# MKimiSH/video-filler

Hardware: AMD Instinct MI355X
Metric: netG+netD fwd+bwd images/sec, 128x128 center-mask (higher is better)
Workload: dtype f32

## Files before the change

video-filler_amd/csrc/vf_conv.hip:

```cpp
#include <algorithm>
#include <vector>
#include <cstdlib>

#include "vf_device.h"

template <int LD>
__device__ __forceinline__ bf16x8 vf_tr_frag(const __bf16* tile, int col0, int k0, int lane) {
  const int grp = lane >> 4, i = lane & 15;
  const __bf16* a = tile + (k0 + 8 * (grp >> 1) + (i >> 2)) * LD + col0 + 16 * (grp & 1) + 4 * (i & 3);
  typedef __attribute__((address_space(3))) bf16x4 lds_bf16x4;
  const bf16x4 lo = __builtin_amdgcn_ds_read_tr16_b64_v4bf16((lds_bf16x4*)a);
  const bf16x4 hi = __builtin_amdgcn_ds_read_tr16_b64_v4bf16((lds_bf16x4*)(a + 4 * LD));
  return __builtin_shufflevector(lo, hi, 0, 1, 2, 3, 4, 5, 6, 7);
}

struct IGemm {
  const float* A;
  const float* Wt;
  const float* bias;
  float* Y;
  float* slab;
  int64_t out_elems;
  unsigned a_bytes, w_bytes;
  int M, lgMh, lgMw;
// ... 1302 lines not shown
  VF_REQUIRE((s.stride == 2 && s.pad == 1) || (s.stride == 1 && s.pad == 0), "unsupported stride/pad %d/%d", s.stride, s.pad);
  VF_REQUIRE(s.B > 0 && s.Cin > 0 && s.Cout > 0, "bad sizes B=%d Cin=%d Cout=%d", s.B, s.Cin, s.Cout);
  VF_REQUIRE(s.pow2_map(), "spatial sizes must be powers of two (got %dx%d)", s.H, s.W);
  if (s.stride == 1) VF_REQUIRE(s.H >= 4 && s.W >= 4, "4x4 stride-1 conv needs H,W >= 4");
  if (s.stride == 2) VF_REQUIRE(s.H >= 2 && s.W >= 2, "stride-2 conv needs H,W >= 2");
  VF_REQUIRE((int64_t)s.Cin * s.Cout * 16 < ((int64_t)1 << 31), "weight tensor too large for 32-bit element offsets");
  return 0;
}
static int check_full_conv_args(const VfConvShape& s) {
  VF_REQUIRE(s.main_net_taps(), "unsupported full-conv shape");
  VF_REQUIRE(s.pow2_map(), "spatial sizes must be powers of two");
  return 0;
}

static int conv_like_fwd(vf_ctx* ctx, const float* A, const float* w, const float* bias, float* Y, const VfConvShape& s, int act,
                         float slope, VfConvExtras* ex) {
  const int B = s.B, Hi = s.H, Wi = s.W, C = s.Cin, N = s.Cout, stride = s.stride, pad = s.pad, Ho = s.out_h(), Wo = s.out_w();
  VF_REQUIRE(vf_is_pow2(Ho) && vf_is_pow2(Wo), "output spatial sizes must be powers of two");
  if (N == 1 && stride == 1 && Hi == 4 && Wi == 4) {
    hipLaunchKernelGGL(k_dot_fwd, dim3(B), dim3(256), 0, ctx->stream, A, w, bias, Y, 16 * C, act, slope);
    VF_LAUNCH_CHECK();
    return 0;
  }
  IGemm g;
  memset(&g, 0, sizeof(g));
  g.A = A; g.Wt = w; g.bias = bias; g.Y = Y;
  g.lgMh = vf_ilog2(Ho); g.lgMw = vf_ilog2(Wo);
  g.M = B * Ho * Wo;
  g.Hi = Hi; g.Wi = Wi; g.C = C; g.N = N;
  g.TH = 4; g.TW = 4;
  g.sy = stride; g.ty = 1; g.oy0 = -pad; g.sx = stride; g.tx = 1; g.ox0 = -pad;
  g.kh0 = 0; g.khs = 1; g.kw0 = 0; g.kws = 1;
  g.wsN = 16 * C; g.wsC = 1; g.wsTap = C;
  g.outH = Ho; g.outW = Wo; g.osy = 1; g.osx = 1;
  g.out_elems = (int64_t)g.M * N;
  g.act = act; g.slope = slope;
  return launch_igemm(ctx, g, (C % 16 == 0) && vf_aligned16(A), (C % 16 == 0) && vf_aligned16(w), ex);
}

static int conv_like_bwd(vf_ctx* ctx, const float* A, const float* w, const float* bias, float* Y, const VfConvShape& s, int act,
                         float slope, VfConvExtras* ex, const float* dmask = nullptr, int dact = 0, float dslope = 0.f) {
  const int B = s.B, Hi = s.H, Wi = s.W, C = s.Cin, N = s.Cout, stride = s.stride, pad = s.pad;
  if (stride == 2 && pad == 1 && N <= 4 && !dmask && !ex->bn.st.mode) {
    const int rc = vf_internal_deconv_thin_out(ctx, A, w, bias, Y, s, act, slope);
    if (rc >= 0) return rc;
  }
  IGemm g;
  memset(&g, 0, sizeof(g));
  g.A = A; g.Wt = w; g.bias = bias; g.Y = Y;
  g.dmask = dmask; g.dact = dact; g.dslope = dslope;
  g.Hi = Hi; g.Wi = Wi; g.C = C; g.N = N;
  g.wsN = 1; g.wsC = 16 * N; g.wsTap = N;
  g.act = act; g.slope = slope;
  const bool vecA = (C % 16 == 0) && vf_aligned16(A);
  bool vecB = (N % 4 == 0) && vf_aligned16(w);
  if (stride == 2 && N < 32 && vecA && vf_aligned16(w) && ctx->ws_front == 0) {
    const int64_t Mi = (int64_t)B * Hi * Wi;
    const size_t col_bytes = (size_t)Mi * 16 * N * sizeof(float);
    if (col_bytes + ((size_t)32 << 20) <= ctx->ws_bytes) {
      float* cols = (float*)ctx->ws;
      ctx->ws_front = (col_bytes + 255) & ~(size_t)255;
      IGemm q;
      memset(&q, 0, sizeof(q));
      q.A = A; q.Wt = w; q.bias = nullptr; q.Y = cols;
      q.M = (int)Mi; q.lgMh = 0; q.lgMw = 0;
      q.Hi = 1; q.Wi = 1; q.C = C; q.N = 16 * N;
      q.TH = 1; q.TW = 1; q.sy = 1; q.ty = 1; q.sx = 1; q.tx = 1; q.khs = 1; q.kws = 1;
      q.wsN = 1; q.wsC = 16 * N; q.wsTap = 0;
      q.outH = 1; q.outW = 1; q.osy = 1; q.osx = 1;
      q.out_elems = Mi * 16 * N;
      q.act = VF_ACT_NONE;
      const int rc = launch_igemm(ctx, q, true, true, nullptr);
      ctx->ws_front = 0;
      if (rc) return rc;
      const int64_t total = Mi * 4 * N;
      VfProf prof(ctx, "col2im4x4", 0.0, 4.0 * ((double)Mi * 16 * N + (double)total));
      hipLaunchKernelGGL(k_col2im4x4, dim3((unsigned)vf_cdiv(total, 256)), dim3(256), 0, ctx->stream, (const float*)cols, bias, Y,
                         B, vf_ilog2(Hi), vf_ilog2(Wi), N, act, slope);
      VF_LAUNCH_CHECK();
      if (dmask) return vf_act_bwd(ctx, dmask, Y, Y, total, dact, dslope);
      return 0;
    }
  }
  if (stride == 2) {
    g.lgMh = vf_ilog2(Hi); g.lgMw = vf_ilog2(Wi);
    g.M = B * Hi * Wi;
    g.TH = 2; g.TW = 2;
    g.sy = 1; g.ty = -1; g.oy0 = 0; g.sx = 1; g.tx = -1; g.ox0 = 0;
    g.khs = 2; g.kws = 2;
    g.outH = 2 * Hi; g.outW = 2 * Wi; g.osy = 2; g.osx = 2;
    g.parity = 1;
    g.out_elems = (int64_t)B * g.outH * g.outW * N;
  } else {
    VF_REQUIRE(Hi == 1 && Wi == 1, "stride-1 transposed pass is built for the 1x1 bottleneck only (got %dx%d)", Hi, Wi);
    g.lgMh = 0; g.lgMw = 0;
    g.M = B;
    g.TH = 1; g.TW = 1;
    g.sy = 1; g.ty = 1; g.sx = 1; g.tx = 1;
    g.N = 16 * N;
    g.wsC = 16 * N; g.wsTap = 0;
    g.outH = 1; g.outW = 1; g.osy = 1; g.osx = 1;
    g.out_elems = (int64_t)B * 16 * N;
    vecB = ((16 * N) % 4 == 0) && vf_aligned16(w);
  }
  VF_REQUIRE(!(dmask && bias), "activation-backward epilogue is for data-gradient passes (no bias)");
  if (stride == 1 && bias) {
    g.bias = nullptr;
    g.act = VF_ACT_NONE;
  }
  if (int rc = launch_igemm(ctx, g, vecA, vecB, stride == 2 ? ex : nullptr)) return rc;
  if (stride == 1 && bias) {
    const int64_t total = (int64_t)B * 16 * N;
    const int nb = (int)std::min<int64_t>(vf_cdiv(total, 256), 4096);
    hipLaunchKernelGGL(k_slab_reduce, dim3(nb), dim3(256), 0, ctx->stream, (const float*)Y, Y, bias, total, N, 0, act, slope, 1.f);
    VF_LAUNCH_CHECK();
  }
  return 0;
}

struct WgRec {
  WGrad g;
  int bm, bf;
  VfPWGrad pw;
  bool plain_ok;
  int blocks;
  int64_t total;
  double flops;
};
struct WgRecorder {
  std::vector<WgRec> recs;
  size_t ws_used = 0;
};
void vf_internal_wg_free(vf_ctx* ctx) {
  delete (WgRecorder*)ctx->wg_rec;
  ctx->wg_rec = nullptr;
}
template <int BM, int BF>
static void launch_wg_group(vf_ctx* ctx, const WGradGroup& G, int blocks, const char* name, double flops) {
  VF_LAUNCH_TIMED(ctx, name, flops, 0.0, (k_wgrad_group<BM, true, true, BF>), dim3(blocks), dim3(256), G);
}
static int wg_flush(vf_ctx* ctx) {
  WgRecorder* R = (WgRecorder*)ctx->wg_rec;
  if (!R || R->recs.empty()) return 0;
  {
    bool any_planes = false;
    for (const WgRec& r : R->recs) any_planes |= (r.bf == 4);
    if (any_planes)
      for (WgRec& r : R->recs)
        if ((r.bf == 3 || r.bf == 1) && r.plain_ok) {
          r.bf = 4;
          r.blocks = r.pw.gx * r.pw.gy;
        }
    VfPWGradGroup G;
    int blocks = 0;
    double fl = 0;
    G.n = 0;
    auto fire = [&]() -> int {
      if (G.n == 0) return 0;
      G.blk_off[G.n] = blocks;
      const int rc = vf_internal_pwgrad_group(ctx, G, blocks, "pwgrad_group_128x128x32", fl);
      G.n = 0;
      blocks = 0;
      fl = 0;
      return rc;
    };
    for (const WgRec& r : R->recs) {
      if (r.bf != 4) continue;
      G.blk_off[G.n] = blocks;
      G.d[G.n] = r.pw;
      ++G.n;
      blocks += (r.blocks + 7) & ~7;
      fl += r.flops;
      if (G.n == VF_PWG_MAX)
        if (int rc = fire()) return rc;
    }
    if (int rc = fire()) return rc;
  }
  for (int bm : {128, 64})
    for (int bf : {3, 1, 0}) {
      WGradGroup G;
      int blocks = 0;
      double fl = 0;
      G.n = 0;
      auto fire = [&]() {
        if (G.n == 0) return;
        G.blk_off[G.n] = blocks;
        char name[64];
        snprintf(name, sizeof(name), "wgrad_group_%dx128%s", bm, bf == 3 ? "_bf16x3" : (bf ? "_bf16" : ""));
        if (bm == 128) {
          if (bf == 3) launch_wg_group<128, 3>(ctx, G, blocks, name, fl);
          else if (bf == 1) launch_wg_group<128, 1>(ctx, G, blocks, name, fl);
          else launch_wg_group<128, 0>(ctx, G, blocks, name, fl);
        } else {
          if (bf == 3) launch_wg_group<64, 3>(ctx, G, blocks, name, fl);
          else if (bf == 1) launch_wg_group<64, 1>(ctx, G, blocks, name, fl);
          else launch_wg_group<64, 0>(ctx, G, blocks, name, fl);
        }
        G.n = 0;
        blocks = 0;
        fl = 0;
      };
      for (const WgRec& r : R->recs) {
        if (r.bm != bm || r.bf != bf) continue;
        G.blk_off[G.n] = blocks;
        G.d[G.n] = r.g;
        ++G.n;
        blocks += (r.blocks + 7) & ~7;
        fl += r.flops;
        if (G.n == VF_WG_GROUP_MAX) fire();
      }
      fire();
    }
  VF_LAUNCH_CHECK();
  {
    SlabGroup S;
    int blocks = 0;
    double bytes = 0;
    S.n = 0;
    auto fire = [&]() {
      if (S.n == 0) return;
      S.blk_off[S.n] = blocks;
      VfProf prof(ctx, "slab_reduce_wgrad_group", 0.0, bytes);
      hipLaunchKernelGGL(k_slab_reduce4_group, dim3(blocks), dim3(256), 0, ctx->stream, S);
      S.n = 0;
      blocks = 0;
      bytes = 0;
    };
    for (const WgRec& r : R->recs) {
      if (r.g.ksplit <= 1) continue;
      S.blk_off[S.n] = blocks;
      S.d[S.n].slab = r.g.slab;
      S.d[S.n].dst = r.g.dW;
      S.d[S.n].total4 = r.total / 4;
      S.d[S.n].ksplit = r.g.ksplit;
      S.d[S.n].beta = r.g.beta;
      ++S.n;
      blocks += (int)vf_cdiv(r.total / 4, 64);
      bytes += 4.0 * (double)r.total * (r.g.ksplit + 1);
      if (S.n == VF_WG_GROUP_MAX) fire();
    }
    fire();
  }
  VF_LAUNCH_CHECK();
  R->recs.clear();
  R->ws_used = 0;
  return 0;
}
VF_API int vf_wgrad_group_begin(vf_ctx* ctx) {
  if (!ctx->wg_rec) ctx->wg_rec = new WgRecorder();
  if (ctx->wg_active) {
    ((WgRecorder*)ctx->wg_rec)->recs.clear();
    ((WgRecorder*)ctx->wg_rec)->ws_used = 0;
  }
  ctx->wg_active = 1;
  return 0;
}
VF_API int vf_wgrad_group_abort(vf_ctx* ctx) {
  if (ctx->wg_rec) {
    ((WgRecorder*)ctx->wg_rec)->recs.clear();
    ((WgRecorder*)ctx->wg_rec)->ws_used = 0;
  }
  ctx->wg_active = 0;
  return 0;
}
VF_API int vf_wgrad_group_end(vf_ctx* ctx) {
  VF_REQUIRE(ctx->wg_active, "vf_wgrad_group_end: no group is open");
  ctx->wg_active = 0;
  return wg_flush(ctx);
}

VF_API int vf_wgrad_group_count(vf_ctx* ctx, int* count) {
  VF_REQUIRE(count != nullptr, "vf_wgrad_group_count: NULL");
  *count = (ctx->wg_active && ctx->wg_rec) ? (int)((WgRecorder*)ctx->wg_rec)->recs.size() : 0;
  return 0;
}
VF_API int vf_wgrad_group_end_partial(vf_ctx* ctx, int count) {
  VF_REQUIRE(ctx->wg_active, "vf_wgrad_group_end_partial: no group is open");
  WgRecorder* R = (WgRecorder*)ctx->wg_rec;
  if (!R || R->recs.empty() || count <= 0) return 0;
  if (count >= (int)R->recs.size()) {
    const size_t used = R->ws_used;
    const int rc = wg_flush(ctx);
    R->ws_used = used;
    return rc;
  }
  std::vector<WgRec> rest(R->recs.begin() + count, R->recs.end());
  R->recs.resize((size_t)count);
  const size_t used = R->ws_used;
  const int rc = wg_flush(ctx);
  R->recs = rest;
  R->ws_used = used;
  return rc;
}

static int wgrad(vf_ctx* ctx, const float* U, const float* V, float* dW, const VfConvShape& s, bool full, float beta, const void* Up,
                 const void* Vp) {
  const int B = s.B, stride = s.stride, pad = s.pad, ntaps = 16;
  const int Hl = full ? s.H : s.out_h(), Wl = full ? s.W : s.out_w(), Nu = full ? s.Cin : s.Cout;
  const int Hv = full ? s.full_out_h() : s.H, Wv = full ? s.full_out_w() : s.W, Cv = full ? s.Cout : s.Cin;
  if (Hl == 1 && Wl == 1 && Hv == 4 && Wv == 4 && stride == 1 && pad == 0 && ntaps == 16) {
    const int rc = vf_internal_wgrad_smallk(ctx, U, V, dW, B, Nu, 16 * Cv, beta);
    if (rc >= 0) return rc;
  }
  WGrad g;
  memset(&g, 0, sizeof(g));
  g.U = U; g.V = V; g.dW = dW;
  g.P = B * Hl * Wl;
  g.lgMh = vf_ilog2(Hl); g.lgMw = vf_ilog2(Wl);
  g.Nu = Nu; g.Cv = Cv; g.Hv = Hv; g.Wv = Wv;
  g.stride = stride; g.pad = pad;
  g.ntaps = ntaps;
  g.nk = (int)vf_cdiv(g.P, ctx->mfma_bf16 ? 32 : 16);
  VF_REQUIRE((int64_t)g.P * Nu < ((int64_t)1 << 29) && (int64_t)B * Hv * Wv * Cv < ((int64_t)1 << 29),
             "operand exceeds the 2 GiB buffer-descriptor range");
  g.u_bytes = (unsigned)((int64_t)g.P * Nu * 4);
  g.v_bytes = (unsigned)((int64_t)B * Hv * Wv * Cv * 4);
  const bool vecU = (Nu % 4 == 0) && vf_aligned16(U);
  const bool vecV = (Cv % 4 == 0) && vf_aligned16(V);
  g.beta = beta;
  const int BM = Nu > 64 ? 128 : 64;
  const int gy = (int)vf_cdiv(Nu, BM), gx = (int)vf_cdiv(ntaps * (int64_t)Cv, 128);
  const int64_t blocks = (int64_t)gx * gy;
  const int64_t total = (int64_t)Nu * ntaps * Cv;
  int ksplit = 1;
  const bool use_pw = Up && Vp && (ctx->mfma_bf16 == 3 || ctx->mfma_bf16 == 1) && ntaps == 16 && stride == 2 && pad == 1 && Nu % 128 == 0 &&
                      Cv % 64 == 0 && g.P % 32 == 0 && (int64_t)g.P * Nu * 6 < ((int64_t)1 << 31) &&
                      (int64_t)B * Hv * Wv * Cv * 6 < ((int64_t)1 << 31) && total % 4 == 0;
  const int wg_blocks = use_pw ? 256 : 512;
  if (blocks < wg_blocks * 3 / 4 && g.nk >= 16) {
    ksplit = (int)std::min<int64_t>(g.nk / 8, vf_cdiv(wg_blocks, blocks));
    while (ksplit > 1 && (size_t)ksplit * total * sizeof(float) > vf_ws_avail(ctx)) --ksplit;
    if (ksplit < 1) ksplit = 1;
    const int steps = (int)vf_cdiv(g.nk, ksplit);
    ksplit = (int)vf_cdiv(g.nk, steps);
  }
  g.ksplit = ksplit;
  g.slab = ksplit > 1 ? (float*)vf_ws_ptr(ctx) : nullptr;
  g.gx = gx; g.gy = gy; g.gz = ksplit;
  dim3 grid((unsigned)gx * gy * ksplit), block(256);
  const bool own_group = use_pw && !ctx->wg_active;
  if (own_group) {
    if (!ctx->wg_rec) ctx->wg_rec = new WgRecorder();
    ctx->wg_active = 1;
  }
  if (ctx->wg_active && (use_pw || (vecU && vecV && (ksplit == 1 || total % 4 == 0)))) {
    WgRecorder* R = (WgRecorder*)ctx->wg_rec;
    const size_t need = ksplit > 1 ? (((size_t)ksplit * total * sizeof(float) + 255) & ~(size_t)255) : 0;
    if (R->ws_used + need > vf_ws_avail(ctx)) {
      if (int rc = wg_flush(ctx)) return rc;
      R->ws_used = 0;
    }
    VF_REQUIRE(need <= vf_ws_avail(ctx), "workspace too small for this layer's split-K slabs");
    if (ksplit > 1) g.slab = (float*)(vf_ws_ptr(ctx) + R->ws_used);
    R->ws_used += need;
    WgRec r;
    r.g = g;
    r.bm = BM;
    r.bf = ctx->mfma_bf16;
    r.blocks = gx * gy * ksplit;
    r.total = total;
    r.flops = 2.0 * (double)g.P * Nu * (double)ntaps * Cv;
    r.plain_ok = false;
    if (!use_pw && (ctx->mfma_bf16 == 3 || ctx->mfma_bf16 == 1) && BM == 128 && ksplit == 1 && Hl == 1 && Wl == 1 && Hv == 4 && Wv == 4 && stride == 1 &&
        pad == 0 && ntaps == 16 && Nu % 4 == 0 && (16 * Cv) % 128 == 0 && vecU && vecV) {
      r.plain_ok = true;
      VfPWGrad& w = r.pw;
      memset(&w, 0, sizeof(w));
      w.Uf = U; w.Vf = V;
      w.out = dW;
      w.P = g.P; w.Nu = Nu; w.Cv = Cv; w.Hv = Hv; w.Wv = Wv;
      w.gx = (16 * Cv) / 128; w.gy = (int)vf_cdiv(Nu, 128); w.gz = 1;
      w.ksplit = 1; w.nk = (int)vf_cdiv(g.P, 32);
      w.beta = beta;
    }
    if (use_pw) {
      r.bf = 4;
      VfPWGrad& w = r.pw;
      memset(&w, 0, sizeof(w));
      w.Up = Up; w.Vp = Vp;
      w.out = ksplit > 1 ? g.slab : dW;
      w.u_ps = (unsigned)((int64_t)g.P * Nu * 2);
      w.v_ps = (unsigned)((int64_t)B * Hv * Wv * Cv * 2);
      w.P = g.P; w.lgMh = g.lgMh; w.lgMw = g.lgMw;
      w.Nu = Nu; w.Cv = Cv; w.Hv = Hv; w.Wv = Wv;
      w.gx = gx; w.gy = gy; w.gz = ksplit;
      w.ksplit = ksplit; w.nk = g.nk;
      w.beta = beta;
    }
    R->recs.push_back(r);
    if (own_group) {
      ctx->wg_active = 0;
      return wg_flush(ctx);
    }
    return 0;
  }
  if (ctx->wg_active) {
    WgRecorder* R = (WgRecorder*)ctx->wg_rec;
    const size_t need = ksplit > 1 ? (((size_t)ksplit * total * sizeof(float) + 255) & ~(size_t)255) : 0;
    if (R && R->ws_used + need <= vf_ws_avail(ctx)) {
      if (ksplit > 1) g.slab = (float*)(vf_ws_ptr(ctx) + R->ws_used);
      R->ws_used += need;
    } else if (int rc = wg_flush(ctx)) {
      return rc;
    }
  }
  {
    const int bf = ctx->mfma_bf16;
    const char* wname = BM == 128 ? (bf == 3 ? "wgrad_128x128_bf16x3" : bf ? "wgrad_128x128_bf16" : "wgrad_128x128")
                                  : (bf == 3 ? "wgrad_64x128_bf16x3" : bf ? "wgrad_64x128_bf16" : "wgrad_64x128");
    const double wfl = 2.0 * (double)g.P * Nu * (double)ntaps * Cv;
#define VF_WG(BM_, BF_)                                                                              \
  do {                                                                                              \
    if (vecU && vecV)                                                                               \
      VF_LAUNCH_TIMED(ctx, wname, wfl, 0.0, (k_wgrad<BM_, true, true, BF_>), grid, block, g);       \
    else if (vecU)                                                                                  \
      VF_LAUNCH_TIMED(ctx, wname, wfl, 0.0, (k_wgrad<BM_, true, false, BF_>), grid, block, g);      \
    else if (vecV)                                                                                  \
      VF_LAUNCH_TIMED(ctx, wname, wfl, 0.0, (k_wgrad<BM_, false, true, BF_>), grid, block, g);      \
    else                                                                                            \
      VF_LAUNCH_TIMED(ctx, wname, wfl, 0.0, (k_wgrad<BM_, false, false, BF_>), grid, block, g);     \
  } while (0)
    if (BM == 128) {
      if (bf == 3) VF_WG(128, 3); else if (bf) VF_WG(128, 1); else VF_WG(128, 0);
    } else {
      if (bf == 3) VF_WG(64, 3); else if (bf) VF_WG(64, 1); else VF_WG(64, 0);
    }
#undef VF_WG
  }
  VF_LAUNCH_CHECK();
  if (ksplit > 1) {
    VfProf prof(ctx, "slab_reduce_wgrad", 0.0, 4.0 * (double)total * (ksplit + 1));
    return launch_slab_reduce(ctx, g.slab, dW, nullptr, total, 1, ksplit, VF_ACT_NONE, 0.f, beta);
  }
  return 0;
}

VF_API int vf_conv_is_fast(int H, int W, int k, int stride, int pad) { return VfConvShape{0, H, W, 0, 0, k, stride, pad}.matrix_core_conv(); }

int vf_internal_conv2d_fwd(vf_ctx* ctx, const float* x, const float* w, const float* bias, float* y, const VfConvShape& s, int act,
                           float slope, VfConvExtras* ex) {
  if (!s.matrix_core_conv()) return vf_internal_gconv_fwd(ctx, x, w, bias, y, s, act, slope);
  if (int rc = check_conv_args(s)) return rc;
  if (s.stride == 2 && s.Cin == 3 && !ex->bn.st.mode) {
    const int rc = vf_internal_conv_thin_fwd(ctx, x, w, bias, y, nullptr, s, act, slope, ex);
    if (rc >= 0) return rc;
  }
  return conv_like_fwd(ctx, x, w, bias, y, s, act, slope, ex);
}
VF_API int vf_conv2d_fwd(vf_ctx* ctx, const float* x, const float* w, const float* bias, float* y, int B, int H, int W,
                         int Cin, int Cout, int k, int stride, int pad, int act, float slope) {
  const VfConvShape s{B, H, W, Cin, Cout, k, stride, pad};
  return vf_take_pending(ctx, [&](VfConvExtras* ex) { return vf_internal_conv2d_fwd(ctx, x, w, bias, y, s, act, slope, ex); });
}

int vf_internal_conv2d_bwd_data(vf_ctx* ctx, const float* gy, const float* w, float* gx, const VfConvShape& s, VfConvExtras* ex) {
  if (!s.matrix_core_conv()) return vf_internal_gconv_bwd_data(ctx, gy, w, gx, s);
  if (int rc = check_conv_args(s)) return rc;
  if (s.stride == 1) {
    VF_REQUIRE(s.H == 4 && s.W == 4, "stride-1 conv data-grad is built for the 4x4 bottleneck input only");
    if (s.Cout == 1) {
      const int64_t n = (int64_t)s.B * 16 * s.Cin;
      hipLaunchKernelGGL(k_dot_bwd_data, dim3((int)vf_cdiv(n, 256)), dim3(256), 0, ctx->stream, gy, w, gx, s.B, 16 * s.Cin, ex->dot_act_y,
                         ex->dot_act, ex->dot_act_slope);
      VF_LAUNCH_CHECK();
      return 0;
    }
  }
  return conv_like_bwd(ctx, gy, w, nullptr, gx, s.gradient_of_conv(), VF_ACT_NONE, 0.f, ex);
}
VF_API int vf_conv2d_bwd_data(vf_ctx* ctx, const float* gy, const float* w, float* gx, int B, int H, int W, int Cin,
                              int Cout, int k, int stride, int pad) {
  const VfConvShape s{B, H, W, Cin, Cout, k, stride, pad};
  return vf_take_pending(ctx, [&](VfConvExtras* ex) { return vf_internal_conv2d_bwd_data(ctx, gy, w, gx, s, ex); });
}

int vf_internal_conv2d_bwd_data_act(vf_ctx* ctx, const float* gy, const float* w, float* gx, const float* x_act, int act, float slope,
                                    const VfConvShape& s, VfConvExtras* ex) {
  if (int rc = check_conv_args(s)) return rc;
  VF_REQUIRE(x_act != nullptr && (act == VF_ACT_LRELU || act == VF_ACT_RELU),
             "vf_conv2d_bwd_data_act: needs the activated input and a (leaky) ReLU");
  VF_REQUIRE(s.stride == 2, "vf_conv2d_bwd_data_act: only the stride-2 layers follow a bare conv + activation pair");
// ... 72 lines not shown
```

video-filler_amd/csrc/vf_pgemm.hip:

```cpp
#include <algorithm>
#include <cstdlib>

#include "vf_device.h"

template <int NPL>
__global__ __launch_bounds__(256) void k_planes_split(const float* __restrict__ x, __bf16* __restrict__ planes, int64_t n4,
                                                      int64_t pstride) {
  for (int64_t i = blockIdx.x * (int64_t)blockDim.x + threadIdx.x; i < n4; i += (int64_t)gridDim.x * blockDim.x) {
    if constexpr (NPL == 1) {
      *(u32x2*)(planes + 4 * i) = vf_round4(((const f32x4*)x)[i]);
    } else {
      u32x2 o[3];
      vf_split3(((const f32x4*)x)[i], o);
#pragma unroll
      for (int q = 0; q < 3; ++q) *(u32x2*)(planes + q * pstride + 4 * i) = o[q];
    }
  }
}
__global__ __launch_bounds__(256) void k_weight_planes(const float* __restrict__ w, __bf16* __restrict__ nat, __bf16* __restrict__ tr,
                                                       int d0, int d1, int64_t pstride, int npl) {
  __shared__ float tile[32][33];
  const int t0 = blockIdx.x * 32, tap = blockIdx.y, u0 = blockIdx.z * 32;
  const int tx = threadIdx.x & 31, ty = threadIdx.x >> 5;
  for (int j = ty; j < 32; j += 8) {
// ... 888 lines not shown
  const int arow = wm + lr;
  int slot_base;
  unsigned tap_ok = 0xffffu;
  int a_col = 0;
  if constexpr (MODE == 0) {
    a_col = arow & 15;
    slot_base = (arow >> 4) * PW + a_col;
  } else {
    const int oy = (arow >> LW) & (Wo - 1), ox = arow & (Wo - 1);
    slot_base = (arow >> (2 * LW)) * HW + (oy - 1 + ph) * Wo + (ox - 1 + pw);
    tap_ok = 0;
#pragma unroll
    for (int s_ = 0; s_ < NS; ++s_) {
      const int di = (TR ? ph : ((s_ >> 3) & 1)) + ((s_ >> 1) & 1) - 1, dj = (TR ? pw : ((s_ >> 2) & 1)) + (s_ & 1) - 1;
      if ((unsigned)(oy + di) < (unsigned)Ho && (unsigned)(ox + dj) < (unsigned)Wo) tap_ok |= 1u << s_;
    }
  }
  const int brow = wn + lr;
  unsigned b_off0 = (unsigned)(brow * 128);
  const unsigned b_sw = (unsigned)((brow >> 1) & 7);

  auto a_addr = [&](auto STEP, unsigned& off, unsigned& sw) {
    constexpr int s_ = decltype(STEP)::value;
    constexpr int cth = TR ? 0 : (s_ >> 3) & 1, ctw = TR ? 0 : (s_ >> 2) & 1, a = (s_ >> 1) & 1, b = s_ & 1;
    if constexpr (MODE == 0) {
      off = (unsigned)((slot_base + a * PW + b) * 128);
      sw = (unsigned)((a_col + b) & 7);
    } else {
      const int raw = slot_base + (cth + a) * Wo + ctw + b;
      const bool ok = (tap_ok >> s_) & 1u;
      off = (unsigned)((ok ? raw : (128 | (raw & 1))) * 128);
      sw = (unsigned)((raw >> 1) & 7);
    }
  };

  bf16x8 lo_held[4];
  auto read_lo_ahead = [&](auto STEP) {
    unsigned off, sw;
    a_addr(STEP, off, sw);
#pragma unroll
    for (int g = 0; g < 4; ++g) lo_held[g] = *(const bf16x8*)(smem + OFF_LO + off + ((((unsigned)(2 * g + lh)) ^ sw) << 4));
  };
  auto compute_step = [&](auto STEP, int pb, int wbuf) {
    constexpr int s_ = decltype(STEP)::value;
    constexpr bool held = (s_ & 3) == 3;
    unsigned a_off, a_sw;
    a_addr(STEP, a_off, a_sw);
    const unsigned char* pa = smem + 2 * pb * PL + a_off;
    const unsigned char* pl = smem + OFF_LO + a_off;
    const unsigned char* wb = smem + OFF_W + wbuf * WBUF + b_off0;
    bf16x8 a[2][3], bb[2][3];
    auto read_frag = [&](int g, int set) {
      const unsigned o = (unsigned)(2 * g + lh);
      a[set][0] = *(const bf16x8*)(pa + ((o ^ a_sw) << 4));
      a[set][1] = *(const bf16x8*)(pa + PL + ((o ^ a_sw) << 4));
      if constexpr (!held) a[set][2] = *(const bf16x8*)(pl + ((o ^ a_sw) << 4));
#pragma unroll
      for (int q = 0; q < 3; ++q) bb[set][q] = *(const bf16x8*)(wb + q * W_PL + ((o ^ b_sw) << 4));
    };
    read_frag(0, 0);
#pragma unroll
    for (int g = 0; g < 4; ++g) {
      const int cs = g & 1;
      if (g + 1 < 4) read_frag(g + 1, cs ^ 1);
      __builtin_amdgcn_sched_barrier(0);
      bf16x8 a2;
      if constexpr (held) a2 = lo_held[g];
      else a2 = a[cs][2];
      acc[0][0] = __builtin_amdgcn_mfma_f32_32x32x16_bf16(a[cs][1], bb[cs][1], acc[0][0], 0, 0, 0);
      acc[0][0] = __builtin_amdgcn_mfma_f32_32x32x16_bf16(a[cs][0], bb[cs][2], acc[0][0], 0, 0, 0);
      acc[0][0] = __builtin_amdgcn_mfma_f32_32x32x16_bf16(a2, bb[cs][0], acc[0][0], 0, 0, 0);
      acc[0][0] = __builtin_amdgcn_mfma_f32_32x32x16_bf16(a[cs][0], bb[cs][1], acc[0][0], 0, 0, 0);
      acc[0][0] = __builtin_amdgcn_mfma_f32_32x32x16_bf16(a[cs][1], bb[cs][0], acc[0][0], 0, 0, 0);
      acc[0][0] = __builtin_amdgcn_mfma_f32_32x32x16_bf16(a[cs][0], bb[cs][0], acc[0][0], 0, 0, 0);
      __builtin_amdgcn_sched_barrier(0);
    }
  };

  auto pix_of = [&](int row) -> int64_t {
    if constexpr (MODE == 0) return ((int64_t)b_img * Ho + oy0 + (row >> 4)) * Wo + ox0 + (row & 15);
    else if constexpr (!TR) return (int64_t)bx * 128 + row;
    else {
      const int img = bx * (128 / HW) + (row >> (2 * LW)), my = (row >> LW) & (Wo - 1), mx = row & (Wo - 1);
      return ((int64_t)img * (2 * Ho) + 2 * my + ph) * (2 * Wo) + 2 * mx + pw;
    }
  };
  float pre_d[16], pre_x[16];
  const bool fin_tile = p.ksplit == 1;
  const bool want_d = fin_tile && p.dmask != nullptr, want_x = fin_tile && p.st.mode == 2;
#pragma unroll
  for (int r = 0; r < 16; ++r) {
    pre_d[r] = 1.f;
    pre_x[r] = 0.f;
  }
  if (want_d || want_x) {
    const int n = n0 + wn + lr;
    const int bw = 2 * (n >> 6) + (n & 1), bb = (n >> 1) & 31, wpp = p.N >> 5;
#pragma unroll
    for (int r = 0; r < 16; ++r) {
      const int64_t pix = pix_of(wm + (r & 3) + 8 * (r >> 2) + 4 * lh);
      if (want_d) pre_d[r] = p.dbits ? (float)((p.dbits[pix * wpp + bw] >> bb) & 1u) : p.dmask[pix * p.N + n];
      if (want_x) pre_x[r] = p.st.x[pix * p.N + n];
    }
  }

  dma_patch_plane(ch0, 0, 0, VfIntC<0>{}, !(p.dbg & 32));
  dma_patch_plane(ch0, 0, 0, VfIntC<1>{}, !(p.dbg & 32));
  dma_patch_plane(ch0, 0, 0, VfIntC<2>{}, !(p.dbg & 32));
  dma_w(ch0, VfIntC<0>{}, 0, !(p.dbg & 32));
  for (int c = 0; c < cps; ++c) {
    const int ch = ch0 + c;
    asm volatile("" : "+v"(slot_base), "+v"(b_off0), "+s"(rowA), "+s"(colA));
    vf_static_for<NS>([&](auto S) {
      constexpr int s_ = decltype(S)::value, cls = s_ >> 2, t = s_ & 3, wbuf = s_ & 1;
      const int pb = TR ? (c & 1) : (cls & 1);
      const bool last_unit = (c + 1 == cps) && (TR || cls == 3);
      const int nch = (TR || cls == 3) ? ch + 1 : ch, ncls = TR ? 0 : ((cls + 1) & 3);
      if constexpr (t == 1 || t == 2) {
        if (last_unit) asm volatile("s_waitcnt vmcnt(0) lgkmcnt(0)" ::: "memory");
        else asm volatile("s_waitcnt vmcnt(2) lgkmcnt(0)" ::: "memory");
      } else {
        asm volatile("s_waitcnt vmcnt(0) lgkmcnt(0)" ::: "memory");
      }
      asm volatile("s_barrier" ::: "memory");
      __builtin_amdgcn_sched_barrier(0);
      if (!(p.dbg & 1)) {
        if constexpr (s_ + 1 < NS) dma_w(ch, VfIntC<s_ + 1>{}, wbuf ^ 1, true);
        else dma_w(ch + 1, VfIntC<0>{}, wbuf ^ 1, c + 1 < cps);
        if constexpr (t == 0) dma_patch_plane(nch, ncls, pb ^ 1, VfIntC<0>{}, !last_unit);
        if constexpr (t == 1) dma_patch_plane(nch, ncls, pb ^ 1, VfIntC<1>{}, !last_unit);
        if constexpr (t == 3) dma_patch_plane(nch, ncls, pb ^ 1, VfIntC<2>{}, !last_unit);
      }
      if constexpr (t == 2) read_lo_ahead(VfIntC<s_ + 1>{});
      __builtin_amdgcn_sched_barrier(0);
      if (!(p.dbg & 4)) compute_step(S, pb, wbuf);
    });
  }
  asm volatile("s_waitcnt vmcnt(0)\n\ts_barrier" ::: "memory");
  typedef const float (&pre_t)[1][16];
  pg_epilogue_at<1, 1, 4, 64, true>(p, acc, red, n0, wm, wn, lane, tid, wave >> 1, bx, ks, ph, pw, true, reinterpret_cast<pre_t>(pre_d),
                                    reinterpret_cast<pre_t>(pre_x), pix_of);
}

__device__ __forceinline__ bf16x8 pg_tr_frag(const __bf16* tile, int col0, int k0, int lane) {
  const int grp = lane >> 4, i = lane & 15;
  const int k = k0 + 8 * (grp >> 1) + (i >> 2);
  const int blk = (col0 >> 5) ^ ((i >> 2) & 3);
  const __bf16* a = tile + k * 128 + blk * 32 + 16 * (grp & 1) + 4 * (i & 3);
  typedef __attribute__((address_space(3))) bf16x4 lds_bf16x4;
  const bf16x4 lo = __builtin_amdgcn_ds_read_tr16_b64_v4bf16((lds_bf16x4*)a);
  const bf16x4 hi = __builtin_amdgcn_ds_read_tr16_b64_v4bf16((lds_bf16x4*)(a + 4 * 128));
  return __builtin_shufflevector(lo, hi, 0, 1, 2, 3, 4, 5, 6, 7);
}

template <int NPL = 3, int FS = 1>
__global__ __launch_bounds__(512, FS == 1 ? 6 : 1) void k_pwgrad_group(const VfPWGradGroup G) {
  int l = 0;
  while (l + 1 < G.n && (int)blockIdx.x >= G.blk_off[l + 1]) ++l;
  const VfPWGrad& p = G.d[l];
  const int local = (int)blockIdx.x - G.blk_off[l];
  const int ntiles = p.gx * p.gy * p.gz;
  if (local >= ntiles) return;
  constexpr int BK = 32, TILE = BK * 128, PL_SZ = 2 * TILE, ST_SZ = NPL * PL_SZ;
  __shared__ __attribute__((aligned(1024))) __bf16 smem[ST_SZ];

  const int tid = threadIdx.x, lane = tid & 63;
  const int wave = __builtin_amdgcn_readfirstlane(tid >> 6);
  const int wm = (wave >> 1) * 32, wn = (wave & 1) * 64;
  const int lid = vf_xcd_remap(local, ntiles);
  const int jx = __builtin_amdgcn_readfirstlane(lid % p.gx), rest = __builtin_amdgcn_readfirstlane(lid / p.gx);
  const int n0 = __builtin_amdgcn_readfirstlane(rest % p.gy) * 128, j0 = jx * 128;
  const int ks = __builtin_amdgcn_readfirstlane(rest / p.gy);
  const int steps = (p.nk + p.ksplit - 1) / p.ksplit;
  const int kt0 = ks * steps, kt1 = min(p.nk, kt0 + steps);

  const int krow = 4 * wave + (lane >> 4);
  const int slot = lane & 15;
  const int chunk = (((slot >> 2) ^ (krow & 3)) << 2) | (slot & 3);
  const unsigned u_off = 2u * (unsigned)(n0 + 8 * chunk);
  const int col = j0 + 8 * chunk;
  const int tap = col / p.Cv, cch = col - tap * p.Cv;
  const int dy = (tap >> 2) - 1, dx = (tap & 3) - 1;
  const int Mw = 1 << p.lgMw, Mh = 1 << p.lgMh;
  const __amdgpu_buffer_rsrc_t rsU = vf_rsrc(p.Up, (unsigned)NPL * p.u_ps), rsV = vf_rsrc(p.Vp, (unsigned)NPL * p.v_ps);
  const unsigned lds0 = (unsigned)(uintptr_t)(__attribute__((address_space(3))) void*)smem;
  const unsigned row_lds = 2u * (unsigned)(4 * wave * 128);
  unsigned szero;
  asm volatile("s_mov_b32 %0, 0" : "=s"(szero));

  auto dma_stage = [&](int kt) {
    const int pix = kt * BK + krow;
    const int mx = pix & (Mw - 1), my = (pix >> p.lgMw) & (Mh - 1), b = pix >> (p.lgMw + p.lgMh);
    const int iy = 2 * my + dy, ix = 2 * mx + dx;
    const bool okv = (unsigned)iy < (unsigned)p.Hv && (unsigned)ix < (unsigned)p.Wv;
    const unsigned uo = u_off + 2u * (unsigned)(pix * p.Nu);
    const unsigned vo = okv ? 2u * (unsigned)(((b * p.Hv + iy) * p.Wv + ix) * p.Cv + cch) : VF_OOB;
    const unsigned base = lds0 + row_lds;
#pragma unroll
    for (int q = 0; q < NPL; ++q) {
      pg_dma16(base + 2u * (unsigned)(q * PL_SZ), uo, rsU, szero + q * p.u_ps);
      pg_dma16(base + 2u * (unsigned)(q * PL_SZ + TILE), vo, rsV, szero + q * p.v_ps);
    }
  };

  const bool fed32 = p.Up == nullptr;
  const int Ncols = 16 * p.Cv;
  auto stage_fp32 = [&](int kt) {
    const int c4 = (tid & 31) * 4;
#pragma unroll
    for (int j = 0; j < 2; ++j) {
      const int k = (tid >> 5) + 16 * j;
      const int pix = kt * BK + k;
      f32x4 u = {0.f, 0.f, 0.f, 0.f}, v = {0.f, 0.f, 0.f, 0.f};
      if (pix < p.P) {
        if (n0 + c4 < p.Nu) u = *(const f32x4*)(p.Uf + (int64_t)pix * p.Nu + n0 + c4);
        v = *(const f32x4*)(p.Vf + (int64_t)pix * Ncols + j0 + c4);
      }
      const int off = k * 128 + (((c4 >> 5) ^ (k & 3)) << 5) + (c4 & 31);
      if constexpr (NPL == 1) {
        *(u32x2*)(smem + off) = vf_round4(u);
        *(u32x2*)(smem + TILE + off) = vf_round4(v);
      } else {
        u32x2 up[3], vp[3];
        vf_split3(u, up);
        vf_split3(v, vp);
#pragma unroll
        for (int q = 0; q < 3; ++q) {
          *(u32x2*)(smem + q * PL_SZ + off) = up[q];
          *(u32x2*)(smem + q * PL_SZ + TILE + off) = vp[q];
        }
      }
    }
  };

  f32x16 acc[2];
#pragma unroll
  for (int nt = 0; nt < 2; ++nt)
#pragma unroll
    for (int r = 0; r < 16; ++r) acc[nt][r] = 0.f;
  auto compute_stage = [&]() {
    const __bf16* base = smem;
    if constexpr (FS == 1) {
#pragma unroll
      for (int g = 0; g < BK / 16; ++g) {
        bf16x8 a1[NPL], b1[NPL][2];
#pragma unroll
        for (int q = 0; q < NPL; ++q) {
          a1[q] = pg_tr_frag(base + q * PL_SZ, wm, 16 * g, lane);
#pragma unroll
          for (int nt = 0; nt < 2; ++nt) b1[q][nt] = pg_tr_frag(base + q * PL_SZ + TILE, wn + 32 * nt, 16 * g, lane);
        }
#pragma unroll
        for (int nt = 0; nt < 2; ++nt) {
          if constexpr (NPL == 3) {
            acc[nt] = __builtin_amdgcn_mfma_f32_32x32x16_bf16(a1[1], b1[1][nt], acc[nt], 0, 0, 0);
            acc[nt] = __builtin_amdgcn_mfma_f32_32x32x16_bf16(a1[0], b1[2][nt], acc[nt], 0, 0, 0);
            acc[nt] = __builtin_amdgcn_mfma_f32_32x32x16_bf16(a1[2], b1[0][nt], acc[nt], 0, 0, 0);
            acc[nt] = __builtin_amdgcn_mfma_f32_32x32x16_bf16(a1[0], b1[1][nt], acc[nt], 0, 0, 0);
            acc[nt] = __builtin_amdgcn_mfma_f32_32x32x16_bf16(a1[1], b1[0][nt], acc[nt], 0, 0, 0);
          }
          acc[nt] = __builtin_amdgcn_mfma_f32_32x32x16_bf16(a1[0], b1[0][nt], acc[nt], 0, 0, 0);
        }
      }
    } else {
    bf16x8 a[2][NPL], b[2][NPL][2];
    auto read_frag = [&](int g, int set) {
#pragma unroll
      for (int q = 0; q < NPL; ++q) {
        a[set][q] = pg_tr_frag(base + q * PL_SZ, wm, 16 * g, lane);
#pragma unroll
        for (int nt = 0; nt < 2; ++nt) b[set][q][nt] = pg_tr_frag(base + q * PL_SZ + TILE, wn + 32 * nt, 16 * g, lane);
      }
    };
    read_frag(0, 0);
#pragma unroll
    for (int g = 0; g < BK / 16; ++g) {
      const int cs = g & 1;
      if (g + 1 < BK / 16) read_frag(g + 1, cs ^ 1);
      __builtin_amdgcn_sched_barrier(0);
#pragma unroll
      for (int nt = 0; nt < 2; ++nt) {
        if constexpr (NPL == 3) {
          acc[nt] = __builtin_amdgcn_mfma_f32_32x32x16_bf16(a[cs][1], b[cs][1][nt], acc[nt], 0, 0, 0);
          acc[nt] = __builtin_amdgcn_mfma_f32_32x32x16_bf16(a[cs][0], b[cs][2][nt], acc[nt], 0, 0, 0);
          acc[nt] = __builtin_amdgcn_mfma_f32_32x32x16_bf16(a[cs][2], b[cs][0][nt], acc[nt], 0, 0, 0);
          acc[nt] = __builtin_amdgcn_mfma_f32_32x32x16_bf16(a[cs][0], b[cs][1][nt], acc[nt], 0, 0, 0);
          acc[nt] = __builtin_amdgcn_mfma_f32_32x32x16_bf16(a[cs][1], b[cs][0][nt], acc[nt], 0, 0, 0);
        }
        acc[nt] = __builtin_amdgcn_mfma_f32_32x32x16_bf16(a[cs][0], b[cs][0][nt], acc[nt], 0, 0, 0);
      }
      __builtin_amdgcn_sched_barrier(0);
    }
    }
  };

  if (fed32) {
    for (int kt = kt0; kt < kt1; ++kt) {
      stage_fp32(kt);
      __syncthreads();
      compute_stage();
      __syncthreads();
    }
  } else {
    for (int kt = kt0; kt < kt1; ++kt) {
      dma_stage(kt);
      asm volatile("s_waitcnt vmcnt(0)\n\ts_barrier" ::: "memory");
      __builtin_amdgcn_sched_barrier(0);
      compute_stage();
      asm volatile("s_barrier" ::: "memory");
    }
  }

  const int lr = lane & 31, lh = lane >> 5;
  const int64_t total = (int64_t)p.Nu * Ncols;
  float* out = p.out + (p.ksplit > 1 ? (int64_t)ks * total : 0);
  const bool acc_old = p.ksplit == 1 && p.beta != 0.f;
#pragma unroll
  for (int r = 0; r < 16; ++r) {
    const int n = n0 + wm + (r & 3) + 8 * (r >> 2) + 4 * lh;
    if (n >= p.Nu) continue;
#pragma unroll
    for (int nt = 0; nt < 2; ++nt) {
      const int64_t idx = (int64_t)n * Ncols + j0 + wn + nt * 32 + lr;
      float v = acc[nt][r];
      if (acc_old) v += p.beta * out[idx];
      out[idx] = v;
    }
// ... 229 lines not shown
```

Before: 22520.

## Route Nu=64 weight-gradient layers through grouped bf16x3 pwgrad kernel with 64-row tile

Extends the grouped plane-based weight-gradient path to layers with 64 output channels by adding a 64x128 tile variant inside k_pwgrad_group, used when bf16x3 MFMA mode is on. Such layers previously fell back to the generic wgrad_group kernel. The ksplit target stays at the larger block count for these layers, and kernel names distinguish the mixed groups. This risks lower per-block MFMA utilisation with only half of the 512-thread block's waves loading U, and it adds a divergent branch in the shared kernel.

```diff
diff --git a/video-filler_amd/csrc/vf_conv.hip b/video-filler_amd/csrc/vf_conv.hip
--- a/video-filler_amd/csrc/vf_conv.hip
+++ b/video-filler_amd/csrc/vf_conv.hip
@@ -1478,14 +1478,16 @@
           r.blocks = r.pw.gx * r.pw.gy;
         }
     VfPWGradGroup G;
-    int blocks = 0;
+    int blocks = 0, n64 = 0;
     double fl = 0;
     G.n = 0;
     auto fire = [&]() -> int {
       if (G.n == 0) return 0;
       G.blk_off[G.n] = blocks;
-      const int rc = vf_internal_pwgrad_group(ctx, G, blocks, "pwgrad_group_128x128x32", fl);
+      const char* name = n64 == 0 ? "pwgrad_group_128x128x32" : (n64 == G.n ? "pwgrad_group_64x128x32" : "pwgrad_group_64+128x128x32");
+      const int rc = vf_internal_pwgrad_group(ctx, G, blocks, name, fl);
       G.n = 0;
+      n64 = 0;
       blocks = 0;
       fl = 0;
       return rc;
@@ -1495,6 +1497,7 @@
       G.blk_off[G.n] = blocks;
       G.d[G.n] = r.pw;
       ++G.n;
+      n64 += r.pw.Up != nullptr && r.pw.Nu == 64;
       blocks += (r.blocks + 7) & ~7;
       fl += r.flops;
       if (G.n == VF_PWG_MAX)
@@ -1649,10 +1652,11 @@
   const int64_t blocks = (int64_t)gx * gy;
   const int64_t total = (int64_t)Nu * ntaps * Cv;
   int ksplit = 1;
-  const bool use_pw = Up && Vp && (ctx->mfma_bf16 == 3 || ctx->mfma_bf16 == 1) && ntaps == 16 && stride == 2 && pad == 1 && Nu % 128 == 0 &&
+  const bool pw64 = Nu == 64 && ctx->mfma_bf16 == 3;
+  const bool use_pw = Up && Vp && (ctx->mfma_bf16 == 3 || ctx->mfma_bf16 == 1) && ntaps == 16 && stride == 2 && pad == 1 && (Nu % 128 == 0 || pw64) &&
                       Cv % 64 == 0 && g.P % 32 == 0 && (int64_t)g.P * Nu * 6 < ((int64_t)1 << 31) &&
                       (int64_t)B * Hv * Wv * Cv * 6 < ((int64_t)1 << 31) && total % 4 == 0;
-  const int wg_blocks = use_pw ? 256 : 512;
+  const int wg_blocks = use_pw && !pw64 ? 256 : 512;
   if (blocks < wg_blocks * 3 / 4 && g.nk >= 16) {
     ksplit = (int)std::min<int64_t>(g.nk / 8, vf_cdiv(wg_blocks, blocks));
     while (ksplit > 1 && (size_t)ksplit * total * sizeof(float) > vf_ws_avail(ctx)) --ksplit;
diff --git a/video-filler_amd/csrc/vf_pgemm.hip b/video-filler_amd/csrc/vf_pgemm.hip
--- a/video-filler_amd/csrc/vf_pgemm.hip
+++ b/video-filler_amd/csrc/vf_pgemm.hip
@@ -1064,6 +1064,90 @@
   const bf16x4 hi = __builtin_amdgcn_ds_read_tr16_b64_v4bf16((lds_bf16x4*)(a + 4 * 128));
   return __builtin_shufflevector(lo, hi, 0, 1, 2, 3, 4, 5, 6, 7);
 }
+__device__ __forceinline__ bf16x8 pg_tr_frag64(const __bf16* tile, int col0, int k0, int lane) {
+  const int grp = lane >> 4, i = lane & 15;
+  const int k = k0 + 8 * (grp >> 1) + (i >> 2);
+  const int blk = (col0 >> 5) ^ ((i >> 3) & 1);
+  const __bf16* a = tile + k * 64 + blk * 32 + 16 * (grp & 1) + 4 * (i & 3);
+  typedef __attribute__((address_space(3))) bf16x4 lds_bf16x4;
+  const bf16x4 lo = __builtin_amdgcn_ds_read_tr16_b64_v4bf16((lds_bf16x4*)a);
+  const bf16x4 hi = __builtin_amdgcn_ds_read_tr16_b64_v4bf16((lds_bf16x4*)(a + 4 * 64));
+  return __builtin_shufflevector(lo, hi, 0, 1, 2, 3, 4, 5, 6, 7);
+}
+
+template <int NPL>
+__device__ __forceinline__ void pwgrad_tile64(const VfPWGrad& p, __bf16* smem, int tid, int lane, int wave, int j0, int ks, int kt0,
+                                              int kt1) {
+  constexpr int BK = 32, TILE_U = BK * 64, TILE_V = BK * 128, PL_SZ = TILE_U + TILE_V;
+  const int wm = (wave >> 2) * 32, wn = (wave & 3) * 32;
+  const int krow = 4 * wave + (lane >> 4);
+  const int slot = lane & 15;
+  const int chunk = (((slot >> 2) ^ (krow & 3)) << 2) | (slot & 3);
+  const int col = j0 + 8 * chunk;
+  const int tap = col / p.Cv, cch = col - tap * p.Cv;
+  const int dy = (tap >> 2) - 1, dx = (tap & 3) - 1;
+  const int krow_u = 8 * (wave & 3) + (lane >> 3);
+  const int slot_u = lane & 7;
+  const int chunk_u = (((slot_u >> 2) ^ ((krow_u >> 1) & 1)) << 2) | (slot_u & 3);
+  const unsigned u_off = 2u * (unsigned)(8 * chunk_u);
+  const int Mw = 1 << p.lgMw, Mh = 1 << p.lgMh;
+  const __amdgpu_buffer_rsrc_t rsU = vf_rsrc(p.Up, (unsigned)NPL * p.u_ps), rsV = vf_rsrc(p.Vp, (unsigned)NPL * p.v_ps);
+  const unsigned lds0 = (unsigned)(uintptr_t)(__attribute__((address_space(3))) void*)smem;
+  const unsigned row_v = 2u * (unsigned)(TILE_U + 4 * wave * 128), row_u = 2u * (unsigned)(8 * (wave & 3) * 64);
+  unsigned szero;
+  asm volatile("s_mov_b32 %0, 0" : "=s"(szero));
+  f32x16 acc;
+#pragma unroll
+  for (int r = 0; r < 16; ++r) acc[r] = 0.f;
+  for (int kt = kt0; kt < kt1; ++kt) {
+    {
+      const int pix = kt * BK + krow;
+      const int mx = pix & (Mw - 1), my = (pix >> p.lgMw) & (Mh - 1), b = pix >> (p.lgMw + p.lgMh);
+      const int iy = 2 * my + dy, ix = 2 * mx + dx;
+      const bool okv = (unsigned)iy < (unsigned)p.Hv && (unsigned)ix < (unsigned)p.Wv;
+      const unsigned vo = okv ? 2u * (unsigned)(((b * p.Hv + iy) * p.Wv + ix) * p.Cv + cch) : VF_OOB;
+      const unsigned uo = u_off + 2u * (unsigned)((kt * BK + krow_u) * 64);
+#pragma unroll
+      for (int q = 0; q < NPL; ++q) {
+        if (wave < 4) pg_dma16(lds0 + row_u + 2u * (unsigned)(q * PL_SZ), uo, rsU, szero + q * p.u_ps);
+        pg_dma16(lds0 + row_v + 2u * (unsigned)(q * PL_SZ), vo, rsV, szero + q * p.v_ps);
+      }
+    }
+    asm volatile("s_waitcnt vmcnt(0)\n\ts_barrier" ::: "memory");
+    __builtin_amdgcn_sched_barrier(0);
+#pragma unroll
+    for (int g = 0; g < BK / 16; ++g) {
+      bf16x8 a1[NPL], b1[NPL];
+#pragma unroll
+      for (int q = 0; q < NPL; ++q) {
+        a1[q] = pg_tr_frag64(smem + q * PL_SZ, wm, 16 * g, lane);
+        b1[q] = pg_tr_frag(smem + q * PL_SZ + TILE_U, wn, 16 * g, lane);
+      }
+      if constexpr (NPL == 3) {
+        acc = __builtin_amdgcn_mfma_f32_32x32x16_bf16(a1[1], b1[1], acc, 0, 0, 0);
+        acc = __builtin_amdgcn_mfma_f32_32x32x16_bf16(a1[0], b1[2], acc, 0, 0, 0);
+        acc = __builtin_amdgcn_mfma_f32_32x32x16_bf16(a1[2], b1[0], acc, 0, 0, 0);
+        acc = __builtin_amdgcn_mfma_f32_32x32x16_bf16(a1[0], b1[1], acc, 0, 0, 0);
+        acc = __builtin_amdgcn_mfma_f32_32x32x16_bf16(a1[1], b1[0], acc, 0, 0, 0);
+      }
+      acc = __builtin_amdgcn_mfma_f32_32x32x16_bf16(a1[0], b1[0], acc, 0, 0, 0);
+    }
+    asm volatile("s_barrier" ::: "memory");
+  }
+  const int lr = lane & 31, lh = lane >> 5;
+  const int Ncols = 16 * p.Cv;
+  const int64_t total = (int64_t)64 * Ncols;
+  float* out = p.out + (p.ksplit > 1 ? (int64_t)ks * total : 0);
+  const bool acc_old = p.ksplit == 1 && p.beta != 0.f;
+#pragma unroll
+  for (int r = 0; r < 16; ++r) {
+    const int n = wm + (r & 3) + 8 * (r >> 2) + 4 * lh;
+    const int64_t idx = (int64_t)n * Ncols + j0 + wn + lr;
+    float v = acc[r];
+    if (acc_old) v += p.beta * out[idx];
+    out[idx] = v;
+  }
+}
 
 template <int NPL = 3, int FS = 1>
 __global__ __launch_bounds__(512, FS == 1 ? 6 : 1) void k_pwgrad_group(const VfPWGradGroup G) {
@@ -1085,6 +1169,12 @@
   const int ks = __builtin_amdgcn_readfirstlane(rest / p.gy);
   const int steps = (p.nk + p.ksplit - 1) / p.ksplit;
   const int kt0 = ks * steps, kt1 = min(p.nk, kt0 + steps);
+  if constexpr (NPL == 3) {
+    if (p.Up != nullptr && p.Nu == 64) {
+      pwgrad_tile64<NPL>(p, smem, tid, lane, wave, j0, ks, kt0, kt1);
+      return;
+    }
+  }
 
   const int krow = 4 * wave + (lane >> 4);
   const int slot = lane & 15;
```

Result: faster. 22810 (median of 6 runs) (+1.3%).
